# jgsimard/big-dreamer

Hardware: AMD Instinct MI355X
Metric: latent transitions/sec (RSSM + imagination) at batch=50 chunk=50 H=15 (higher is better)
Workload: dtype f32

## Files before the change

### big_dreamer_amd/csrc/wgrad.hip

```cpp
#include "bd_device.h"
#include "bd_host.h"
#include <stdint.h>
#include <stdlib.h>

namespace bd {

typedef float floatx16 __attribute__((ext_vector_type(16)));
constexpr int kWT = 64;
constexpr int kWM = 32;

__global__ __launch_bounds__(kThreads) void wgrad_kernel(const float* __restrict__ dpre, int ldp,
                                                         const float* __restrict__ act, int lda, int M, int N, int K,
                                                         int has_bias, int rows_per_split, float* __restrict__ ws) {
    __shared__ float P[kWM][kWT];
    __shared__ float A[kWM][kWT];
    const int Kext = K + has_bias;
    const int n0 = blockIdx.x * kWT, k0 = blockIdx.y * kWT;
    const int m_begin = blockIdx.z * rows_per_split;
    const int m_end = min(M, m_begin + rows_per_split);
    const int lane = threadIdx.x & 63, wave = threadIdx.x >> 6;
    const int wn = (wave >> 1) * 32, wk = (wave & 1) * 32;
    floatx16 acc;
#pragma unroll
    for (int i = 0; i < 16; ++i) acc[i] = 0.f;
    const int c = threadIdx.x & 63, r0 = threadIdx.x >> 6;
    for (int m0 = m_begin; m0 < m_end; m0 += kWM) {
        float pv[kWM / 4], av[kWM / 4];
#pragma unroll
        for (int i = 0; i < kWM / 4; ++i) {
            const int m = m0 + r0 + 4 * i;
            const bool ok = m < m_end;
            pv[i] = (ok && n0 + c < N) ? dpre[(size_t)m * ldp + n0 + c] : 0.f;
            const int k = k0 + c;
            av[i] = ok ? (k < K ? act[(size_t)m * lda + k] : (k == K && has_bias ? 1.f : 0.f)) : 0.f;
        }
        __syncthreads();
#pragma unroll
        for (int i = 0; i < kWM / 4; ++i) {
            P[r0 + 4 * i][c] = pv[i];
            A[r0 + 4 * i][c] = av[i];
        }
        __syncthreads();
#pragma unroll
        for (int s = 0; s < kWM / 2; ++s) {
            const float a = P[2 * s + (lane >> 5)][wn + (lane & 31)];
            const float b = A[2 * s + (lane >> 5)][wk + (lane & 31)];
            acc = __builtin_amdgcn_mfma_f32_32x32x2f32(a, b, acc, 0, 0, 0);
        }
    }
    float* slab = ws + (size_t)blockIdx.z * N * Kext;
    const int k = k0 + wk + (lane & 31);
#pragma unroll
    for (int reg = 0; reg < 16; ++reg) {
        const int n = n0 + wn + (reg & 3) + 8 * (reg >> 2) + 4 * (lane >> 5);
        if (n < N && k < Kext) slab[(size_t)n * Kext + k] = acc[reg];
    }
}

__global__ __launch_bounds__(256) void wgrad_reduce_kernel(const float* __restrict__ ws, int splits, int N, int K,
                                                           int has_bias, float* __restrict__ dW, int ldw,
                                                           float* __restrict__ db, int accumulate) {
    const int Kext = K + has_bias;
    const int total = N * Kext;
    for (int e = blockIdx.x * blockDim.x + threadIdx.x; e < total; e += gridDim.x * blockDim.x) {
        float s = 0.f;
        for (int z = 0; z < splits; ++z) s += ws[(size_t)z * total + e];
        const int n = e / Kext, k = e - n * Kext;
        float* dst = k < K ? dW + (size_t)n * ldw + k : db + n;
        *dst = accumulate ? *dst + s : s;
    }
}

__global__ __launch_bounds__(kThreads) void wgrad_grouped_kernel(const bd_wgrad_desc* __restrict__ descs, int n,
                                                                 float* __restrict__ ws) {
    __shared__ float P[kWM][kWT];
    __shared__ float A[kWM][kWT];
    int g = 0;
    while (g + 1 < n && (int)blockIdx.x >= descs[g + 1].block_begin) ++g;
    const bd_wgrad_desc d = descs[g];
    const int hb = d.db != nullptr;
    const int Kext = d.K + hb;
    int local = blockIdx.x - d.block_begin;
    const int z = local / (d.tiles_n * d.tiles_k);
    local -= z * d.tiles_n * d.tiles_k;
    const int n0 = (local / d.tiles_k) * kWT, k0 = (local % d.tiles_k) * kWT;
    const int m_begin = z * d.rows_per;
    const int m_end = min(d.M, m_begin + d.rows_per);
    const int lane = threadIdx.x & 63, wave = threadIdx.x >> 6;
    const int wn = (wave >> 1) * 32, wk = (wave & 1) * 32;
    floatx16 acc;
#pragma unroll
    for (int i = 0; i < 16; ++i) acc[i] = 0.f;
    const int c = threadIdx.x & 63, r0 = threadIdx.x >> 6;
    float pv[kWM / 4], av[kWM / 4];
    auto fetch = [&](int m0) {
#pragma unroll
        for (int i = 0; i < kWM / 4; ++i) {
            const int m = m0 + r0 + 4 * i;
            const bool ok = m < m_end;
            pv[i] = (ok && n0 + c < d.N) ? d.dpre[(size_t)m * d.ldp + n0 + c] : 0.f;
            const int k = k0 + c;
            float v = 0.f;
            if (ok) {
                if (k < d.K) v = m < d.M1 ? d.act1[(size_t)m * d.lda1 + k] : d.act2[(size_t)(m - d.M1) * d.lda2 + k];
                else if (k == d.K && hb) v = 1.f;
            }
            av[i] = v;
        }
    };
    fetch(m_begin);
    for (int m0 = m_begin; m0 < m_end; m0 += kWM) {
        __syncthreads();
#pragma unroll
        for (int i = 0; i < kWM / 4; ++i) {
            P[r0 + 4 * i][c] = pv[i];
            A[r0 + 4 * i][c] = av[i];
        }
        __syncthreads();
        if (m0 + kWM < m_end) fetch(m0 + kWM);
#pragma unroll
        for (int s = 0; s < kWM / 2; ++s) {
            const float a = P[2 * s + (lane >> 5)][wn + (lane & 31)];
            const float b = A[2 * s + (lane >> 5)][wk + (lane & 31)];
            acc = __builtin_amdgcn_mfma_f32_32x32x2f32(a, b, acc, 0, 0, 0);
        }
    }
    float* slab = ws + d.ws_off + (size_t)z * d.N * Kext;
    const int k = k0 + wk + (lane & 31);
#pragma unroll
    for (int reg = 0; reg < 16; ++reg) {
        const int nn = n0 + wn + (reg & 3) + 8 * (reg >> 2) + 4 * (lane >> 5);
        if (nn < d.N && k < Kext) slab[(size_t)nn * Kext + k] = acc[reg];
    }
}

constexpr int kWB = 13;
constexpr int kWBK = 12;
constexpr int kWBKDeep = 36;
__host__ __device__ __forceinline__ int wgrad_tiles_k(int NB, int KB, bool deep_ok) {
    if (KB <= kWB) return 1;
    return (NB <= 4 && deep_ok) ? cdiv(KB, kWBKDeep) : cdiv(KB, kWBK);
}
__host__ inline bool wgrad_act16(const bd_wgrad_desc& d) {
    auto al16 = [](const void* q) { return (reinterpret_cast<uintptr_t>(q) & 15) == 0; };
    if ((d.K & 3) != 0 || !al16(d.act1)) return false;
    if (d.g_nseg > 0) return (d.g_C & 3) == 0 && (d.g_seglen & 3) == 0;
    return (d.lda1 & 3) == 0 && (d.M1 == d.M || ((d.lda2 & 3) == 0 && al16(d.act2)));
}
constexpr int kWLd = 240;
constexpr int kWRows = 16;
constexpr int kWStage = 2 * kWRows * kWLd;
constexpr int kWRing = 3;
constexpr int kWRowsTall = 32;
constexpr int kWLdNarrow = 80;
constexpr int kWLdMid = 144;
constexpr int kWLdDeep = 592;
constexpr size_t kWideLdsBytes = 147456;
static_assert((size_t)kWRing * kWRows * (kWLdNarrow + kWLdDeep) * sizeof(float) <= kWideLdsBytes, "deep stage ring");
static_assert((size_t)kWRing * kWRowsTall * (kWLdMid + kWLd) * sizeof(float) <= kWideLdsBytes, "mid stage ring");
constexpr int kWThreads = 512;

template <int WN, int WK, int ROWS = kWRows, int PLD = kWLd, int ALD = kWLd>
__device__ __forceinline__ void wgrad_wide_body(const bd_wgrad_desc& d, float* __restrict__ ws, float* wlds, int hb, int Kext,
                                                int z, int n0, int k0, int nb_cnt, int kb_cnt) {
    const int m_begin = z * d.rows_per;
    const int m_end = min(d.M, m_begin + d.rows_per);
    const int lane = threadIdx.x & 63;
    const int wave = __builtin_amdgcn_readfirstlane(threadIdx.x >> 6);
    const int wr = wave & 1, wc = wave >> 1;
    const int hn = (nb_cnt + 1) >> 1;
    const int my_nb0 = wr ? hn : 0, my_nb = wr ? nb_cnt - hn : hn;
    const int kq = kb_cnt >> 2, krem = kb_cnt & 3;
    const int my_kb0 = wc * kq + min(wc, krem), my_kb = kq + (wc < krem ? 1 : 0);

    constexpr int kStage = ROWS * (PLD + ALD);
    constexpr int kRpw = ROWS / 8;
    static_assert(kWRing * kStage * sizeof(float) <= kWideLdsBytes, "stage ring exceeds the LDS request");
    floatx4 acc[WN][WK];
#pragma unroll
    for (int i = 0; i < WN; ++i)
#pragma unroll
        for (int j = 0; j < WK; ++j) acc[i][j] = floatx4{0.f, 0.f, 0.f, 0.f};

    typedef __attribute__((address_space(3))) void* lds_ptr_t;
    typedef const __attribute__((address_space(1))) void* glb_ptr_t;
    const int ncol = min(nb_cnt * 16, d.N - n0), kcol = min(kb_cnt * 16, d.K - k0);
    for (int i = threadIdx.x; i < kWRing * kStage; i += kWThreads) wlds[i] = 0.f;
    __syncthreads();
    if (hb && d.K >= k0 && d.K < k0 + kb_cnt * 16 && threadIdx.x < kWRing * ROWS)
        wlds[(threadIdx.x / ROWS) * kStage + ROWS * PLD + (threadIdx.x % ROWS) * ALD + (d.K - k0)] = 1.f;
    auto al16 = [](const void* q) { return (reinterpret_cast<uintptr_t>(q) & 15) == 0; };
    const bool p4 = (ncol & 3) == 0 && (d.ldp & 3) == 0 && al16(d.dpre + n0);
    const bool gathered = d.g_nseg > 0;
    const bool a4 = (kcol & 3) == 0 && (k0 & 3) == 0 &&
                    (gathered ? ((d.g_C & 3) == 0 && (d.g_seglen & 3) == 0 && al16(d.act1))
                              : ((d.lda1 & 3) == 0 && al16(d.act1) && (d.M1 == d.M || ((d.lda2 & 3) == 0 && al16(d.act2)))));
    constexpr int kCh4 = (ALD + 255) / 256;
    constexpr int kCh1 = (ALD + 63) / 64;
    constexpr int kGo = kCh1;
    int goff[kGo];
#pragma unroll
    for (int cc = 0; cc < kGo; ++cc) goff[cc] = 0;
    if (gathered) {
#pragma unroll
        for (int cc = 0; cc < kGo; ++cc) {
            const int k = k0 + (a4 ? 4 * lane + 256 * cc : lane + 64 * cc), sgm = k / d.g_seglen;
            goff[cc] = sgm * d.g_IW * d.g_C + (k - sgm * d.g_seglen);
        }
    }
    auto issue = [&](float* buf, int m0) {
#pragma unroll
        for (int rr = 0; rr < kRpw; ++rr) {
            const int m = m0 + wave * kRpw + rr;
            float* P = buf + (wave * kRpw + rr) * PLD;
            float* A = buf + ROWS * PLD + (wave * kRpw + rr) * ALD;
            if (m < m_end) {
                const float* prow = d.dpre + (size_t)m * d.ldp + n0;
                if (p4) {
                    if (4 * lane < ncol) __builtin_amdgcn_global_load_lds((glb_ptr_t)(prow + 4 * lane), (lds_ptr_t)P, 16, 0, 0);
                } else {
#pragma unroll
                    for (int cc = 0; cc < 4; ++cc) {
                        const int c = lane + 64 * cc;
                        if (c < ncol) __builtin_amdgcn_global_load_lds((glb_ptr_t)(prow + c), (lds_ptr_t)(P + 64 * cc), 4, 0, 0);
                    }
                }
                const float* abase;
                if (gathered) {
                    const int img = m / (d.g_gh * d.g_gw), rem = m - img * d.g_gh * d.g_gw;
                    const int y = rem / d.g_gw, x = rem - y * d.g_gw;
                    abase = d.act1 + (((size_t)img * d.g_IH + 2 * y) * d.g_IW + 2 * x) * d.g_C;
                } else {
                    abase = (m < d.M1 ? d.act1 + (size_t)m * d.lda1 : d.act2 + (size_t)(m - d.M1) * d.lda2) + k0;
                }
                if (a4) {
#pragma unroll
                    for (int cc = 0; cc < kCh4; ++cc)
                        if (4 * lane + 256 * cc < kcol)
                            __builtin_amdgcn_global_load_lds((glb_ptr_t)(abase + (gathered ? goff[cc] : 4 * lane + 256 * cc)),
                                                             (lds_ptr_t)(A + 256 * cc), 16, 0, 0);
                } else {
#pragma unroll
                    for (int cc = 0; cc < kCh1; ++cc) {
                        const int c = lane + 64 * cc;
                        if (c < kcol)
                            __builtin_amdgcn_global_load_lds((glb_ptr_t)(abase + (gathered ? goff[cc] : c)), (lds_ptr_t)(A + 64 * cc), 4,
                                                             0, 0);
                    }
                }
            } else {
#pragma unroll
                for (int cc = 0; cc < kCh1; ++cc) {
                    const int c = lane + 64 * cc;
                    if (c < PLD) P[c] = 0.f;
                    if (c < ALD) A[c] = 0.f;
                }
            }
        }
    };
    const int nst = cdiv(m_end - m_begin, ROWS);
    const int n_dma = kRpw * ((p4 ? 1 : cdiv(ncol, 64)) + (a4 ? cdiv(kcol, 256) : cdiv(kcol, 64)));
    auto wait_keep_newest = [&]() {
        switch (n_dma) {
            case 4: asm volatile("s_waitcnt vmcnt(4)" ::: "memory"); break;
            case 6: asm volatile("s_waitcnt vmcnt(6)" ::: "memory"); break;
            case 8: asm volatile("s_waitcnt vmcnt(8)" ::: "memory"); break;
            case 10: asm volatile("s_waitcnt vmcnt(10)" ::: "memory"); break;
            case 12: asm volatile("s_waitcnt vmcnt(12)" ::: "memory"); break;
            case 14: asm volatile("s_waitcnt vmcnt(14)" ::: "memory"); break;
            default: asm volatile("s_waitcnt vmcnt(16)" ::: "memory"); break;
        }
    };
    __syncthreads();
    issue(wlds, m_begin);
    if (nst > 1) issue(wlds + kStage, m_begin + ROWS);
    __builtin_amdgcn_s_waitcnt(0);
    __syncthreads();
    const int lrow = lane >> 4, lcol = lane & 15;
    for (int st = 0; st < nst; ++st) {
        const float* buf = wlds + (st % kWRing) * kStage;
        const bool more = st + 2 < nst;
        [[maybe_unused]] const int sb = (st == 10 || st == 11) ? (st - 10) * 8 : -1;
        BD_DSTAMP(sb, 0);
        if (more) issue(wlds + ((st + 2) % kWRing) * kStage, m_begin + (st + 2) * ROWS);
        BD_DSTAMP(sb, 1);
        const float* Pb = buf + lrow * PLD + my_nb0 * 16 + lcol;
        const float* Ab = buf + ROWS * PLD + lrow * ALD + my_kb0 * 16 + lcol;
#pragma unroll
        for (int sl = 0; sl < ROWS / 4; ++sl) {
            float a[WN], b[WK];
#pragma unroll
            for (int i = 0; i < WN; ++i) a[i] = Pb[sl * 4 * PLD + i * 16];
#pragma unroll
            for (int j = 0; j < WK; ++j) b[j] = Ab[sl * 4 * ALD + j * 16];
#pragma unroll
            for (int i = 0; i < WN; ++i)
#pragma unroll
                for (int j = 0; j < WK; ++j) acc[i][j] = mfma16(a[i], b[j], acc[i][j]);
        }
        BD_DSTAMP(sb, 2);
        if (more && st + 3 < nst) wait_keep_newest();
        else asm volatile("s_waitcnt vmcnt(0)" ::: "memory");
        BD_DSTAMP(sb, 3);
        lds_barrier();
        BD_DSTAMP(sb, 4);
    }
    float* slab = ws + d.ws_off + (size_t)z * d.N * Kext;
#pragma unroll
    for (int i = 0; i < WN; ++i) {
        if (i < my_nb) {
#pragma unroll
            for (int j = 0; j < WK; ++j) {
                if (j < my_kb) {
                    const int k = k0 + (my_kb0 + j) * 16 + lcol;
#pragma unroll
                    for (int r = 0; r < 4; ++r) {
                        const int nn = n0 + (my_nb0 + i) * 16 + 4 * lrow + r;
                        if (nn < d.N && k < Kext) slab[(size_t)nn * Kext + k] = acc[i][j][r];
                    }
                }
            }
        }
    }
}

template <int WN, int WK>
__device__ __forceinline__ void wgrad_dense_body(const bd_wgrad_desc& d, float* __restrict__ ws, float* wlds, int hb, int Kext,
                                                 int z, int n0, int k0, int nb_cnt, int kb_cnt, int my_nb0, int my_kb0) {
    const int m_begin = z * d.rows_per;
    const int m_end = min(d.M, m_begin + d.rows_per);
    const int lane = threadIdx.x & 63;
    const int wave = __builtin_amdgcn_readfirstlane(threadIdx.x >> 6);
    floatx4 acc[WN][WK];
#pragma unroll
    for (int i = 0; i < WN; ++i)
#pragma unroll
        for (int j = 0; j < WK; ++j) acc[i][j] = floatx4{0.f, 0.f, 0.f, 0.f};
    typedef __attribute__((address_space(3))) void* lds_ptr_t;
    typedef const __attribute__((address_space(1))) void* glb_ptr_t;
    const int ncol = min(nb_cnt * 16, d.N - n0), kcol = min(kb_cnt * 16, d.K - k0);
    for (int i = threadIdx.x; i < kWRing * kWStage; i += kWThreads) wlds[i] = 0.f;
    __syncthreads();
    if (hb && d.K >= k0 && d.K < k0 + kb_cnt * 16 && threadIdx.x < kWRing * kWRows)
        wlds[(threadIdx.x >> 4) * kWStage + kWRows * kWLd + (threadIdx.x & 15) * kWLd + (d.K - k0)] = 1.f;
    const bool lp = 4 * lane < ncol, la = 4 * lane < kcol;
    const float* __restrict__ pl = d.dpre + n0 + 4 * lane;
    const float* __restrict__ a1l = d.act1 + k0 + 4 * lane;
    const float* __restrict__ a2l = (d.M1 < d.M ? d.act2 : d.act1) + k0 + 4 * lane;
    auto issue = [&](float* buf, int m0) {
#pragma unroll
        for (int rr = 0; rr < 2; ++rr) {
            const int m = m0 + wave * 2 + rr;
            float* P = buf + (wave * 2 + rr) * kWLd;
            float* A = P + kWRows * kWLd;
            if (m < m_end) {
                if (lp) __builtin_amdgcn_global_load_lds((glb_ptr_t)(pl + (size_t)m * d.ldp), (lds_ptr_t)P, 16, 0, 0);
                const float* ar = m < d.M1 ? a1l + (size_t)m * d.lda1 : a2l + (size_t)(m - d.M1) * d.lda2;
                if (la) __builtin_amdgcn_global_load_lds((glb_ptr_t)ar, (lds_ptr_t)A, 16, 0, 0);
            } else {
#pragma unroll
                for (int cc = 0; cc < 4; ++cc) {
                    const int c = lane + 64 * cc;
                    if (c < kWLd) {
                        P[c] = 0.f;
                        A[c] = 0.f;
                    }
                }
            }
        }
    };
    const int nst = cdiv(m_end - m_begin, kWRows);
    __syncthreads();
    issue(wlds, m_begin);
    if (nst > 1) issue(wlds + kWStage, m_begin + kWRows);
    __builtin_amdgcn_s_waitcnt(0);
    __syncthreads();
    const int lrow = lane >> 4, lcol = lane & 15;
    for (int st = 0; st < nst; ++st) {
        const float* buf = wlds + (st % kWRing) * kWStage;
        const bool more = st + 2 < nst;
        [[maybe_unused]] const int sb = (st == 10 || st == 11) ? (st - 10) * 8 : -1;
        BD_DSTAMP(sb, 0);
        if (more && wave < 4) issue(wlds + ((st + 2) % kWRing) * kWStage, m_begin + (st + 2) * kWRows);
        BD_DSTAMP(sb, 1);
        const float* Pb = buf + lrow * kWLd + my_nb0 * 16 + lcol;
        const float* Ab = buf + kWRows * kWLd + lrow * kWLd + my_kb0 * 16 + lcol;
#pragma unroll
        for (int sl = 0; sl < kWRows / 4; ++sl) {
            float a[WN], b[WK];
#pragma unroll
            for (int i = 0; i < WN; ++i) a[i] = Pb[sl * 4 * kWLd + i * 16];
#pragma unroll
            for (int j = 0; j < WK; ++j) b[j] = Ab[sl * 4 * kWLd + j * 16];
#pragma unroll
            for (int i = 0; i < WN; ++i)
#pragma unroll
                for (int j = 0; j < WK; ++j) acc[i][j] = mfma16(a[i], b[j], acc[i][j]);
            if (sl == 1 && more && wave >= 4) issue(wlds + ((st + 2) % kWRing) * kWStage, m_begin + (st + 2) * kWRows);
        }
        BD_DSTAMP(sb, 2);
        if (more && st + 3 < nst) asm volatile("s_waitcnt vmcnt(4)" ::: "memory");
        else asm volatile("s_waitcnt vmcnt(0)" ::: "memory");
        BD_DSTAMP(sb, 3);
        lds_barrier();
        BD_DSTAMP(sb, 4);
    }
    float* slab = ws + d.ws_off + (size_t)z * d.N * Kext;
#pragma unroll
    for (int i = 0; i < WN; ++i) {
#pragma unroll
        for (int j = 0; j < WK; ++j) {
            const int k = k0 + (my_kb0 + j) * 16 + lcol;
#pragma unroll
            for (int r = 0; r < 4; ++r) {
                const int nn = n0 + (my_nb0 + i) * 16 + 4 * lrow + r;
                if (nn < d.N && k < Kext) slab[(size_t)nn * Kext + k] = acc[i][j][r];
            }
        }
    }
}

constexpr int kThinMaxKB = 7;
constexpr int kThinDpreFloats = 1024;
__host__ __device__ inline int thin_band_floats(int k, int roww) { return (k * roww + 64 + 255) & ~255; }
__host__ inline bool wgrad_thin_ok(const bd_wgrad_desc& d) {
    auto al16 = [](const void* q) { return (reinterpret_cast<uintptr_t>(q) & 15) == 0; };
    if (d.g_nseg <= 0 || d.g_C > 4 || d.N != 32 || d.ldp != 32 || d.g_gw > 32) return false;
    if (cdiv(d.K, 16) > kThinMaxKB || d.g_seglen != d.g_nseg * d.g_C) return false;
    const int roww = d.g_IW * d.g_C;
    if ((roww & 3) != 0 || !al16(d.act1) || !al16(d.dpre)) return false;
    const size_t per_wave = 2 * (size_t)(thin_band_floats(d.g_nseg, roww) + kThinDpreFloats) * sizeof(float);
    return 8 * per_wave <= kWideLdsBytes && (size_t)8 * 2 * kThinMaxKB * 1024 <= kWideLdsBytes;
}

#ifndef BD_WGRAD_TALL_MID
#define BD_WGRAD_TALL_MID 1
#endif
__device__ __forceinline__ bool tall_mid() { return BD_WGRAD_TALL_MID != 0; }

template <int KB>
__device__ __forceinline__ void wgrad_thin_body(const bd_wgrad_desc& d, float* __restrict__ ws, float* wlds, int z) {
    typedef __attribute__((address_space(3))) void* lds_ptr_t;
    typedef const __attribute__((address_space(1))) void* glb_ptr_t;
    const int lane = threadIdx.x & 63;
    const int wave = __builtin_amdgcn_readfirstlane(threadIdx.x >> 6);
    const int hb = d.db != nullptr;
    const int Kext = d.K + hb;
    const int gh = d.g_gh, gw = d.g_gw, C = d.g_C, kk = d.g_nseg;
    const int roww = d.g_IW * C, band = kk * roww, drow = gw * 32;
    const int band_al = thin_band_floats(kk, roww);
    const int per_buf = band_al + kThinDpreFloats;
    float* mine = wlds + (size_t)wave * 2 * per_buf;
    for (int i = lane; i < 2 * per_buf; i += 64) mine[i] = 0.f;
    asm volatile("s_waitcnt lgkmcnt(0)" ::: "memory");
    const int imgs = d.M / (gh * gw), ipw = d.rows_per / (gh * gw);
    const int img0 = z * ipw, img1 = min(imgs, img0 + ipw);
    const int items = (img1 - img0) * gh;
    const int nband = cdiv(band, 256), ndrow = cdiv(drow, 256);
    auto issue = [&](int it, float* buf) {
        const int img = img0 + it / gh, y = it - (it / gh) * gh;
        const float* sb = d.act1 + ((size_t)img * d.g_IH + 2 * y) * roww;
        const float* sd = d.dpre + ((size_t)img * gh + y) * gw * 32;
        for (int ch = 0; ch < nband; ++ch)
            if (4 * lane + 256 * ch < band)
                __builtin_amdgcn_global_load_lds((glb_ptr_t)(sb + 4 * lane + 256 * ch), (lds_ptr_t)(buf + 256 * ch), 16, 0, 0);
        for (int ch = 0; ch < ndrow; ++ch)
            if (4 * lane + 256 * ch < drow)
                __builtin_amdgcn_global_load_lds((glb_ptr_t)(sd + 4 * lane + 256 * ch), (lds_ptr_t)(buf + band_al + 256 * ch), 16, 0, 0);
    };
    const int n_dma = nband + ndrow;
    auto wait_keep_newest = [&]() {
        switch (n_dma) {
            case 5: asm volatile("s_waitcnt vmcnt(5)" ::: "memory"); break;
            case 6: asm volatile("s_waitcnt vmcnt(6)" ::: "memory"); break;
            case 7: asm volatile("s_waitcnt vmcnt(7)" ::: "memory"); break;
            case 8: asm volatile("s_waitcnt vmcnt(8)" ::: "memory"); break;
            case 9: asm volatile("s_waitcnt vmcnt(9)" ::: "memory"); break;
            case 10: asm volatile("s_waitcnt vmcnt(10)" ::: "memory"); break;
            default: asm volatile("s_waitcnt vmcnt(0)" ::: "memory"); break;
        }
    };
    int boff[KB];
    bool bok[KB];
#pragma unroll
    for (int kb = 0; kb < KB; ++kb) {
        const int kidx = kb * 16 + (lane & 15);
        bok[kb] = kidx < d.K;
        const int ky = kidx / d.g_seglen;
        boff[kb] = bok[kb] ? ky * roww + (kidx - ky * d.g_seglen) : 0;
    }
    floatx4 acc[2][KB];
#pragma unroll
    for (int i = 0; i < 2; ++i)
#pragma unroll
        for (int j = 0; j < KB; ++j) acc[i][j] = floatx4{0.f, 0.f, 0.f, 0.f};
    float bsum[2] = {0.f, 0.f};
    const int q = lane >> 4, n = lane & 15;
    const int nsl = cdiv(gw, 4);
    int it = wave, b = 0;
    if (it < items) issue(it, mine);
    for (; it < items; it += 8, b ^= 1) {
        const bool more = it + 8 < items;
        if (more) {
            issue(it + 8, mine + (b ^ 1) * per_buf);
            wait_keep_newest();
        } else {
            asm volatile("s_waitcnt vmcnt(0)" ::: "memory");
        }
        const float* Bd = mine + b * per_buf;
        const float* Dp = Bd + band_al;
        for (int sl = 0; sl < nsl; ++sl) {
            const int x = 4 * sl + q;
            const float a0 = Dp[x * 32 + n], a1 = Dp[x * 32 + 16 + n];
            float bv[KB];
#pragma unroll
            for (int kb = 0; kb < KB; ++kb) bv[kb] = bok[kb] ? Bd[boff[kb] + 2 * x * C] : 0.f;
#pragma unroll
            for (int kb = 0; kb < KB; ++kb) {
                acc[0][kb] = mfma16(a0, bv[kb], acc[0][kb]);
                acc[1][kb] = mfma16(a1, bv[kb], acc[1][kb]);
            }
            bsum[0] += a0;
            bsum[1] += a1;
        }
        asm volatile("s_waitcnt lgkmcnt(0)" ::: "memory");
    }
    __syncthreads();
    floatx4* R4 = reinterpret_cast<floatx4*>(wlds);
    float* BS = wlds + (size_t)8 * 2 * KB * 256;
#pragma unroll
    for (int i = 0; i < 2; ++i) {
#pragma unroll
        for (int j = 0; j < KB; ++j) R4[((wave * 2 + i) * KB + j) * 64 + lane] = acc[i][j];
        BS[(wave * 2 + i) * 64 + lane] = bsum[i];
    }
    __syncthreads();
    float* slab = ws + d.ws_off + (size_t)z * d.N * Kext;
    for (int e = threadIdx.x; e < 2 * KB * 64; e += blockDim.x) {
        const int blk = e >> 6, l = e & 63;
        floatx4 s4 = floatx4{0.f, 0.f, 0.f, 0.f};
        for (int w = 0; w < 8; ++w) s4 += R4[(w * 2 * KB + blk) * 64 + l];
        const int i = blk / KB, j = blk - i * KB;
        const int k = j * 16 + (l & 15);
        if (k < d.K) {
#pragma unroll
            for (int r = 0; r < 4; ++r) slab[(size_t)(i * 16 + 4 * (l >> 4) + r) * Kext + k] = s4[r];
        }
    }
    if (hb && threadIdx.x < 32) {
        const int i = threadIdx.x >> 4, nn = threadIdx.x & 15;
        float t = 0.f;
        for (int w = 0; w < 8; ++w)
            for (int qq = 0; qq < 4; ++qq) t += BS[(w * 2 + i) * 64 + qq * 16 + nn];
        slab[(size_t)(i * 16 + nn) * Kext + d.K] = t;
    }
}

__global__ __launch_bounds__(kWThreads) void wgrad_wide_kernel(const bd_wgrad_desc* __restrict__ descs, int n,
                                                         float* __restrict__ ws) {
    extern __shared__ float wlds[];
    int g = 0;
    while (g + 1 < n && (int)blockIdx.x >= descs[g + 1].block_begin) ++g;
    const bd_wgrad_desc d = descs[g];
    const int hb = d.db != nullptr;
    const int Kext = d.K + hb;
    const int NB = cdiv(d.N, 16), KB = cdiv(Kext, 16);
    const int nbw = cdiv(NB, d.tiles_n), kbw = cdiv(KB, d.tiles_k);
    int local = blockIdx.x - d.block_begin;
    const int z = local / (d.tiles_n * d.tiles_k);
    local -= z * d.tiles_n * d.tiles_k;
    const int tn = local / d.tiles_k, tk = local - tn * d.tiles_k;
    const int n0 = tn * nbw * 16, k0 = tk * kbw * 16;
    const int nb_cnt = min(nbw, NB - tn * nbw), kb_cnt = min(kbw, KB - tk * kbw);
    if (d.g_pad == 1) {
        const int kb_t = cdiv(d.K, 16);
        if (kb_t <= 3) wgrad_thin_body<3>(d, ws, wlds, z);
        else wgrad_thin_body<kThinMaxKB>(d, ws, wlds, z);
        return;
    }
    const int hn = (nb_cnt + 1) >> 1, hk = (kb_cnt + 3) >> 2;
    {
        auto al16 = [](const void* q) { return (reinterpret_cast<uintptr_t>(q) & 15) == 0; };
        const int ncol = min(nb_cnt * 16, d.N - n0), kcol = min(kb_cnt * 16, d.K - k0);
        const bool dense = nb_cnt == 13 && kb_cnt >= 4 && d.g_nseg == 0 && (ncol & 3) == 0 && (d.ldp & 3) == 0 &&
                           al16(d.dpre + n0) && (kcol & 3) == 0 && (k0 & 3) == 0 && (d.lda1 & 3) == 0 && al16(d.act1) &&
                           (d.M1 == d.M || ((d.lda2 & 3) == 0 && al16(d.act2)));
        if (dense) {
            const int wave = __builtin_amdgcn_readfirstlane(threadIdx.x >> 6);
            const int wr = (0xB2 >> wave) & 1;
            const int c = (0x13232100 >> (4 * wave)) & 3;
            const int kq = kb_cnt >> 2, krem = kb_cnt & 3;
            const int my_nb0 = wr ? 7 : 0, my_nb = wr ? 6 : 7;
            const int my_kb0 = c * kq + min(c, krem), my_kb = kq + (c < krem ? 1 : 0);
#define BD_WD(WN, WK) wgrad_dense_body<WN, WK>(d, ws, wlds, hb, Kext, z, n0, k0, nb_cnt, kb_cnt, my_nb0, my_kb0)
#define BD_WD_ROW(WN)                 \
    do {                              \
        if (my_kb == 4) BD_WD(WN, 4); \
        else if (my_kb == 3) BD_WD(WN, 3); \
        else if (my_kb == 2) BD_WD(WN, 2); \
        else BD_WD(WN, 1);            \
    } while (0)
            if (my_nb == 7) BD_WD_ROW(7);
            else BD_WD_ROW(6);
#undef BD_WD_ROW
#undef BD_WD
            return;
        }
    }
    if (nb_cnt <= 4) {
#define BD_WN_BODY(WN, WK) wgrad_wide_body<WN, WK, kWRowsTall, kWLdNarrow>(d, ws, wlds, hb, Kext, z, n0, k0, nb_cnt, kb_cnt)
#define BD_WN_ROW(WN)                      \
    do {                                   \
        if (hk <= 1) BD_WN_BODY(WN, 1);    \
        else if (hk <= 2) BD_WN_BODY(WN, 2); \
        else if (hk <= 3) BD_WN_BODY(WN, 3); \
        else BD_WN_BODY(WN, 4);            \
    } while (0)
        if (kb_cnt > 15) {
#define BD_WDEEP(WN, WK) wgrad_wide_body<WN, WK, kWRows, kWLdNarrow, kWLdDeep>(d, ws, wlds, hb, Kext, z, n0, k0, nb_cnt, kb_cnt)
            if (hn <= 1) { if (hk <= 8) BD_WDEEP(1, 8); else BD_WDEEP(1, 9); }
            else { if (hk <= 8) BD_WDEEP(2, 8); else BD_WDEEP(2, 9); }
#undef BD_WDEEP
            return;
        }
        if (hn <= 1) BD_WN_ROW(1);
        else BD_WN_ROW(2);
#undef BD_WN_ROW
#undef BD_WN_BODY
        return;
    }
    if (nb_cnt <= 8 && tall_mid()) {
#define BD_WM_BODY(WN, WK) wgrad_wide_body<WN, WK, kWRowsTall, kWLdMid>(d, ws, wlds, hb, Kext, z, n0, k0, nb_cnt, kb_cnt)
#define BD_WM_ROW(WN)                      \
    do {                                   \
        if (hk <= 1) BD_WM_BODY(WN, 1);    \
        else if (hk <= 2) BD_WM_BODY(WN, 2); \
        else if (hk <= 3) BD_WM_BODY(WN, 3); \
        else BD_WM_BODY(WN, 4);            \
    } while (0)
        if (hn <= 2) BD_WM_ROW(2);
        else BD_WM_ROW(4);
#undef BD_WM_ROW
#undef BD_WM_BODY
        return;
    }
#define BD_WG_BODY(WN, WK) wgrad_wide_body<WN, WK>(d, ws, wlds, hb, Kext, z, n0, k0, nb_cnt, kb_cnt)
#define BD_WG_ROW(WN)                      \
    do {                                   \
        if (hk <= 1) BD_WG_BODY(WN, 1);    \
        else if (hk <= 2) BD_WG_BODY(WN, 2); \
        else if (hk <= 3) BD_WG_BODY(WN, 3); \
        else BD_WG_BODY(WN, 4);            \
    } while (0)
    if (hn <= 1) BD_WG_ROW(1);
    else if (hn <= 2) BD_WG_ROW(2);
    else if (hn <= 4) BD_WG_ROW(4);
    else BD_WG_ROW(7);
#undef BD_WG_ROW
#undef BD_WG_BODY
}

__global__ __launch_bounds__(256) void wgrad_grouped_reduce_kernel(const bd_wgrad_desc* __restrict__ descs, int n,
                                                                   const float* __restrict__ ws) {
    int g = 0;
    while (g + 1 < n && (int)blockIdx.x >= descs[g + 1].red_begin) ++g;
    const bd_wgrad_desc d = descs[g];
    const int hb = d.db != nullptr;
    const int Kext = d.K + hb;
    const int total = d.N * Kext;
    const int e = (blockIdx.x - d.red_begin) * blockDim.x + threadIdx.x;
    if (e >= total) return;
    const float* p = ws + d.ws_off + e;
    float s = 0.f;
    for (int z = 0; z < d.splits; ++z) s += p[(size_t)z * total];
    const int nn = e / Kext, k = e - nn * Kext;
    if (k < d.K) d.dW[(size_t)nn * d.ldw + k] = s;
    else d.db[nn] = s;
}

#ifdef BD_STAMPS
extern "C" int bd_debug_wstamps(unsigned long long* out64) {
    return hipMemcpyFromSymbol(out64, HIP_SYMBOL(g_dstamps), sizeof(unsigned long long) * 64) == hipSuccess ? 0 : -1;
}
#endif

static bool wgrad_wide() {
    static const char* e = getenv("BD_WGRAD_WIDE");
    return !(e && e[0] == '0');
}
static bool thin_on() {
    static const char* e = getenv("BD_WGRAD_THIN");
    return !(e && e[0] == '0');
}
static int wgrad_rows() {
    static const char* e = getenv("BD_WGRAD_ROWS");
    const int r = e ? atoi(e) : 0;
    return r >= kWRows ? cdiv(r, kWRows) * kWRows : 0;
}

static void wgrad_plan(int M, int N, int K, int has_bias, int* splits, int* rows_per) {
    const int tiles = cdiv(N, kWT) * cdiv(K + has_bias, kWT);
    int s = 1024 / tiles;
    const int max_s = cdiv(M, 2 * kWM);
    if (s > max_s) s = max_s;
    if (s < 1) s = 1;
    int rp = cdiv(cdiv(M, s), kWM) * kWM;
    *rows_per = rp;
    *splits = cdiv(M, rp);
}

}

extern "C" {

int bd_wgrad_plan(bd_wgrad_desc* descs, int n, int* total_blocks, int* total_red_blocks, size_t* ws_floats) {
    using namespace bd;
    BD_REQUIRE(descs && n > 0 && total_blocks && total_red_blocks && ws_floats, "bd_wgrad_plan: bad arguments");
    int blocks = 0, red = 0;
    size_t off = 0;
    int rows_wide = wgrad_rows();
    if (wgrad_wide() && rows_wide == 0) {
        auto wgs = [&](int R) {
            long t = 0;
            for (int i = 0; i < n; ++i)
                t += (long)cdiv(cdiv(descs[i].N, 16), kWB) * wgrad_tiles_k(cdiv(descs[i].N, 16), cdiv(descs[i].K + (descs[i].db != nullptr), 16), wgrad_act16(descs[i])) *
                     cdiv(descs[i].M > 0 ? descs[i].M : 1, R);
            return t;
        };
        rows_wide = 128;
        while (wgs(rows_wide) > 256 && rows_wide < (1 << 20)) rows_wide += kWRows;
    }
    bool any_gather = false;
    for (int i = 0; i < n; ++i) any_gather = any_gather || descs[i].g_nseg > 0;
    auto tile_cost = [](int nb, int kb) {
        const int hn = (nb + 1) >> 1, kq = kb >> 2, kr = kb & 3;
        const int c = hn * ((kq + (0 < kr ? 1 : 0)) + (kq + (2 < kr ? 1 : 0)));
        return (c > 0 ? c : 1) + 12;
    };
    auto desc_geo = [&](const bd_wgrad_desc& d, int* tiles, int* cost) {
        const int NB = cdiv(d.N, 16), KB = cdiv(d.K + (d.db != nullptr), 16);
        const int tn = cdiv(NB, kWB), tk = wgrad_tiles_k(NB, KB, wgrad_act16(d));
        *tiles = tn * tk;
        *cost = tile_cost(cdiv(NB, tn), cdiv(KB, tk));
    };
    auto thin = [&](const bd_wgrad_desc& d) { return wgrad_wide() && thin_on() && wgrad_thin_ok(d); };
    auto rows_for = [&](const bd_wgrad_desc& d, double T) {
        int t, c;
        desc_geo(d, &t, &c);
        long r = (long)(T / c);
        r = (r / kWRows) * kWRows;
        return (int)(r < 4 * kWRows ? 4 * kWRows : (r > (1 << 22) ? (1 << 22) : r));
    };
    auto blocks_for = [&](double T) {
        long b = 0;
        for (int i = 0; i < n; ++i) {
            const bd_wgrad_desc& d = descs[i];
            if (thin(d)) {
                const int imgs = d.M / (d.g_gh * d.g_gw);
                b += cdiv(imgs, cdiv(imgs, 256));
                continue;
            }
            int t, c;
            desc_geo(d, &t, &c);
            b += (long)t * cdiv(d.M > 0 ? d.M : 1, rows_for(d, T));
        }
        return b;
    };
    double budget = 0.0;
    if (wgrad_wide() && any_gather) {
        double W = 0.0;
        for (int i = 0; i < n; ++i) {
            int t, c;
            desc_geo(descs[i], &t, &c);
            W += (double)t * (descs[i].M > 0 ? descs[i].M : 1) * c;
        }
        double R = W / (256.0 * 1024.0 * 61.0);
        if (R < 1.0) R = 1.0;
        if (R > 24.0) R = 24.0;
        const int rounds = (int)(R + 0.999);
        budget = W / (256.0 * (double)rounds);
        long target = 256L * rounds;
        if (blocks_for(budget * 8.0) > target) target += 256;
        for (int it = 0; it < 200 && blocks_for(budget) > target; ++it) budget *= 1.02;
    }
    for (int i = 0; i < n; ++i) {
        bd_wgrad_desc& d = descs[i];
        BD_REQUIRE(d.dpre && d.act1 && d.dW && d.M > 0 && d.N > 0 && d.K > 0 && d.M1 >= 0 && d.M1 <= d.M,
                   "bd_wgrad_plan: descriptor %d is malformed", i);
        BD_REQUIRE(d.M1 == d.M || d.act2, "bd_wgrad_plan: descriptor %d needs a second activation source", i);
        BD_REQUIRE(d.ldp >= d.N && (d.g_nseg > 0 || d.lda1 >= d.K) && d.ldw >= d.K && (d.M1 == d.M || d.lda2 >= d.K),
                   "bd_wgrad_plan: descriptor %d has a leading dimension that is too small", i);
        if (d.g_nseg > 0)
            BD_REQUIRE(wgrad_wide() && d.M1 == d.M && d.g_seglen > 0 && d.g_nseg * d.g_seglen == d.K && d.g_gh > 0 &&
                           d.g_gw > 0 && d.M % (d.g_gh * d.g_gw) == 0 && d.g_C > 0 && 2 * (d.g_gh - 1) + d.g_nseg <= d.g_IH &&
                           (2 * (d.g_gw - 1)) * d.g_C + d.g_seglen <= d.g_IW * d.g_C,
                       "bd_wgrad_plan: descriptor %d has an inconsistent gather geometry", i);
        const int hb = d.db != nullptr;
        d.g_pad = 0;
        if (wgrad_wide() && wgrad_thin_ok(d) && thin_on()) {
            const int px = d.g_gh * d.g_gw, imgs = d.M / px;
            const int ipw = cdiv(imgs, 256);
            d.g_pad = 1;
            d.tiles_n = d.tiles_k = 1;
            d.rows_per = ipw * px;
            d.splits = cdiv(imgs, ipw);
        } else if (wgrad_wide()) {
            d.tiles_n = cdiv(cdiv(d.N, 16), kWB);
            d.tiles_k = wgrad_tiles_k(cdiv(d.N, 16), cdiv(d.K + hb, 16), wgrad_act16(d));
            d.rows_per = rows_wide;
            if (budget > 0.0) d.rows_per = rows_for(d, budget);
            d.splits = cdiv(d.M, d.rows_per);
        } else {
            d.tiles_n = cdiv(d.N, kWT);
            d.tiles_k = cdiv(d.K + hb, kWT);
            int s = d.M / 512;
            if (s < 1) s = 1;
            if (s > 64) s = 64;
            d.rows_per = cdiv(cdiv(d.M, s), kWM) * kWM;
            d.splits = cdiv(d.M, d.rows_per);
        }
        d.block_begin = blocks;
        d.red_begin = red;
        d.ws_off = off;
        blocks += d.tiles_n * d.tiles_k * d.splits;
        red += cdiv(d.N * (d.K + hb), 256);
        off += (size_t)d.splits * d.N * (d.K + hb);
    }
    *total_blocks = blocks;
    *total_red_blocks = red;
    *ws_floats = off;
    return 0;
}

int bd_wgrad_grouped(const bd_wgrad_desc* descs_dev, int n, int total_blocks, int total_red_blocks, float* ws,
                     void* stream) {
    return bd_wgrad_grouped_phase(descs_dev, n, total_blocks, total_red_blocks, ws, 0, stream);
}

int bd_wgrad_grouped_phase(const bd_wgrad_desc* descs_dev, int n, int total_blocks, int total_red_blocks, float* ws,
                           int phase, void* stream) {
    using namespace bd;
    BD_REQUIRE(descs_dev && ws && n > 0 && n <= 4096 && total_blocks > 0 && total_red_blocks > 0 && phase >= 0 && phase <= 2,
               "bd_wgrad_grouped: bad arguments");
    if (phase == 2) {
    } else if (wgrad_wide()) {
        static_assert(kThreads == 256, "the 64x64-tile wgrad kernels are written for four waves");
        static bool lds_ok = false;
        if (!lds_ok) {
            if (allow_big_lds(wgrad_wide_kernel)) return -1;
            lds_ok = true;
        }
        hipLaunchKernelGGL(wgrad_wide_kernel, dim3(total_blocks), dim3(kWThreads), kWideLdsBytes, (hipStream_t)stream,
                           descs_dev, n, ws);
    } else {
        hipLaunchKernelGGL(wgrad_grouped_kernel, dim3(total_blocks), dim3(kThreads), 0, (hipStream_t)stream, descs_dev, n, ws);
    }
    BD_CHECK_LAUNCH("bd_wgrad_grouped");
    if (phase == 1) return 0;
    hipLaunchKernelGGL(wgrad_grouped_reduce_kernel, dim3(total_red_blocks), dim3(256), 0, (hipStream_t)stream, descs_dev, n,
                       ws);
    BD_CHECK_LAUNCH("bd_wgrad_grouped(reduce)");
    return 0;
}

size_t bd_wgrad_ws_floats(int M, int N, int K) {
    int s0, s1, rp;
    bd::wgrad_plan(M, N, K, 0, &s0, &rp);
    bd::wgrad_plan(M, N, K, 1, &s1, &rp);
    const size_t a = (size_t)s0 * N * K, b = (size_t)s1 * N * (K + 1);
    return a > b ? a : b;
}

int bd_wgrad(const float* dpre, int ldp, const float* act, int lda, int M, int N, int K, float* dW, int ldw,
             float* db, int accumulate, float* ws, size_t ws_floats, void* stream) {
    using namespace bd;
    BD_REQUIRE(dpre && act && dW && ws && M > 0 && N > 0 && K > 0, "bd_wgrad: bad arguments");
    BD_REQUIRE(ldp >= N && lda >= K && ldw >= K, "bd_wgrad: leading dimension too small");
    const int hb = db != nullptr;
    int splits, rows_per;
    wgrad_plan(M, N, K, hb, &splits, &rows_per);
    BD_REQUIRE((size_t)splits * N * (K + hb) <= ws_floats, "bd_wgrad: workspace too small (%zu floats, need %zu)",
               ws_floats, (size_t)splits * N * (K + hb));
    hipLaunchKernelGGL(wgrad_kernel, dim3(cdiv(N, kWT), cdiv(K + hb, kWT), splits), dim3(kThreads), 0,
                       (hipStream_t)stream, dpre, ldp, act, lda, M, N, K, hb, rows_per, ws);
    BD_CHECK_LAUNCH("bd_wgrad");
    const int total = N * (K + hb);
    hipLaunchKernelGGL(wgrad_reduce_kernel, dim3(cdiv(total, 256) < 1024 ? cdiv(total, 256) : 1024), dim3(256), 0,
                       (hipStream_t)stream, ws, splits, N, K, hb, dW, ldw, db, accumulate);
    BD_CHECK_LAUNCH("bd_wgrad(reduce)");
    return 0;
}

}
```

Before: 13.47 million.

## Pad wgrad split slabs, vectorize stores and reduce, and allow multi-round row splits

```diff
diff --git a/big_dreamer_amd/csrc/wgrad.hip b/big_dreamer_amd/csrc/wgrad.hip
--- a/big_dreamer_amd/csrc/wgrad.hip
+++ b/big_dreamer_amd/csrc/wgrad.hip
@@ -159,6 +159,9 @@
 static_assert((size_t)kWRing * kWRows * (kWLdNarrow + kWLdDeep) * sizeof(float) <= kWideLdsBytes, "deep stage ring");
 static_assert((size_t)kWRing * kWRowsTall * (kWLdMid + kWLd) * sizeof(float) <= kWideLdsBytes, "mid stage ring");
 constexpr int kWThreads = 512;
+__host__ __device__ __forceinline__ int wgrad_pitch(int Kext) { return (Kext + 3) & ~3; }
+constexpr int kWMaxRounds = 3;
+constexpr int kWUnitFloor = 256;
 
 template <int WN, int WK, int ROWS = kWRows, int PLD = kWLd, int ALD = kWLd>
 __device__ __forceinline__ void wgrad_wide_body(const bd_wgrad_desc& d, float* __restrict__ ws, float* wlds, int hb, int Kext,
@@ -305,7 +308,8 @@
         lds_barrier();
         BD_DSTAMP(sb, 4);
     }
-    float* slab = ws + d.ws_off + (size_t)z * d.N * Kext;
+    const int pitch = wgrad_pitch(Kext);
+    float* slab = ws + d.ws_off + (size_t)z * d.N * pitch;
 #pragma unroll
     for (int i = 0; i < WN; ++i) {
         if (i < my_nb) {
@@ -316,7 +320,7 @@
 #pragma unroll
                     for (int r = 0; r < 4; ++r) {
                         const int nn = n0 + (my_nb0 + i) * 16 + 4 * lrow + r;
-                        if (nn < d.N && k < Kext) slab[(size_t)nn * Kext + k] = acc[i][j][r];
+                        if (nn < d.N && k < Kext) slab[(size_t)nn * pitch + k] = acc[i][j][r];
                     }
                 }
             }
@@ -339,10 +343,6 @@
     typedef __attribute__((address_space(3))) void* lds_ptr_t;
     typedef const __attribute__((address_space(1))) void* glb_ptr_t;
     const int ncol = min(nb_cnt * 16, d.N - n0), kcol = min(kb_cnt * 16, d.K - k0);
-    for (int i = threadIdx.x; i < kWRing * kWStage; i += kWThreads) wlds[i] = 0.f;
-    __syncthreads();
-    if (hb && d.K >= k0 && d.K < k0 + kb_cnt * 16 && threadIdx.x < kWRing * kWRows)
-        wlds[(threadIdx.x >> 4) * kWStage + kWRows * kWLd + (threadIdx.x & 15) * kWLd + (d.K - k0)] = 1.f;
     const bool lp = 4 * lane < ncol, la = 4 * lane < kcol;
     const float* __restrict__ pl = d.dpre + n0 + 4 * lane;
     const float* __restrict__ a1l = d.act1 + k0 + 4 * lane;
@@ -370,9 +370,23 @@
         }
     };
     const int nst = cdiv(m_end - m_begin, kWRows);
-    __syncthreads();
     issue(wlds, m_begin);
     if (nst > 1) issue(wlds + kWStage, m_begin + kWRows);
+    {
+        const int one = (hb && d.K >= k0 && d.K < k0 + kb_cnt * 16) ? d.K - k0 : -1;
+        const int npad = nb_cnt * 16 - ncol, pad = npad + kb_cnt * 16 - kcol;
+        for (int i = threadIdx.x; i < kWRing * kWRows * pad; i += kWThreads) {
+            const int row = i / pad, c = i - row * pad;
+            float* P = wlds + (row >> 4) * kWStage + (row & 15) * kWLd;
+            if (c < npad) {
+                P[ncol + c] = 0.f;
+            } else {
+                const int kc = kcol + c - npad;
+                const bool live = row >= 2 * kWRows || m_begin + row < m_end;
+                P[kWRows * kWLd + kc] = (kc == one && live) ? 1.f : 0.f;
+            }
+        }
+    }
     __builtin_amdgcn_s_waitcnt(0);
     __syncthreads();
     const int lrow = lane >> 4, lcol = lane & 15;
@@ -405,18 +419,27 @@
         lds_barrier();
         BD_DSTAMP(sb, 4);
     }
-    float* slab = ws + d.ws_off + (size_t)z * d.N * Kext;
+    const int pitch = wgrad_pitch(Kext);
+    float* slab = ws + d.ws_off + (size_t)z * d.N * pitch;
+    constexpr int kFl = WK * 16 + 4;
+    constexpr int kQ = WK * 4;
+    float* mine = wlds + wave * (16 * (4 * 16 + 4));
+    const int kw0 = k0 + my_kb0 * 16;
 #pragma unroll
     for (int i = 0; i < WN; ++i) {
 #pragma unroll
-        for (int j = 0; j < WK; ++j) {
-            const int k = k0 + (my_kb0 + j) * 16 + lcol;
-#pragma unroll
-            for (int r = 0; r < 4; ++r) {
-                const int nn = n0 + (my_nb0 + i) * 16 + 4 * lrow + r;
-                if (nn < d.N && k < Kext) slab[(size_t)nn * Kext + k] = acc[i][j][r];
-            }
-        }
+        for (int j = 0; j < WK; ++j)
+#pragma unroll
+            for (int r = 0; r < 4; ++r) mine[(4 * lrow + r) * kFl + j * 16 + lcol] = acc[i][j][r];
+        asm volatile("s_waitcnt lgkmcnt(0)" ::: "memory");
+#pragma unroll
+        for (int t = 0; t < WK; ++t) {
+            const int idx = t * 64 + lane, row = idx / kQ, q = idx - row * kQ;
+            const floatx4 v = *reinterpret_cast<const floatx4*>(mine + row * kFl + 4 * q);
+            const int nn = n0 + (my_nb0 + i) * 16 + row, k = kw0 + 4 * q;
+            if (nn < d.N && k < pitch) *reinterpret_cast<floatx4*>(slab + (size_t)nn * pitch + k) = v;
+        }
+        asm volatile("s_waitcnt lgkmcnt(0)" ::: "memory");
     }
 }
 
@@ -535,7 +558,8 @@
         BS[(wave * 2 + i) * 64 + lane] = bsum[i];
     }
     __syncthreads();
-    float* slab = ws + d.ws_off + (size_t)z * d.N * Kext;
+    const int pitch = wgrad_pitch(Kext);
+    float* slab = ws + d.ws_off + (size_t)z * d.N * pitch;
     for (int e = threadIdx.x; e < 2 * KB * 64; e += blockDim.x) {
         const int blk = e >> 6, l = e & 63;
         floatx4 s4 = floatx4{0.f, 0.f, 0.f, 0.f};
@@ -544,7 +568,7 @@
         const int k = j * 16 + (l & 15);
         if (k < d.K) {
 #pragma unroll
-            for (int r = 0; r < 4; ++r) slab[(size_t)(i * 16 + 4 * (l >> 4) + r) * Kext + k] = s4[r];
+            for (int r = 0; r < 4; ++r) slab[(size_t)(i * 16 + 4 * (l >> 4) + r) * pitch + k] = s4[r];
         }
     }
     if (hb && threadIdx.x < 32) {
@@ -552,7 +576,7 @@
         float t = 0.f;
         for (int w = 0; w < 8; ++w)
             for (int qq = 0; qq < 4; ++qq) t += BS[(w * 2 + i) * 64 + qq * 16 + nn];
-        slab[(size_t)(i * 16 + nn) * Kext + d.K] = t;
+        slab[(size_t)(i * 16 + nn) * pitch + d.K] = t;
     }
 }
 
@@ -678,6 +702,36 @@
     else d.db[nn] = s;
 }
 
+constexpr int kRedWideThreads = 64;
+constexpr int kRedFly = 16;
+__global__ __launch_bounds__(kRedWideThreads) void wgrad_wide_reduce_kernel(const bd_wgrad_desc* __restrict__ descs, int n,
+                                                                            const float* __restrict__ ws) {
+    int g = 0;
+    while (g + 1 < n && (int)blockIdx.x >= descs[g + 1].red_begin) ++g;
+    const bd_wgrad_desc d = descs[g];
+    const int hb = d.db != nullptr;
+    const int q4 = wgrad_pitch(d.K + hb) >> 2;
+    const int total4 = d.N * q4;
+    const int e = (blockIdx.x - d.red_begin) * kRedWideThreads + threadIdx.x;
+    if (e >= total4) return;
+    const floatx4* p = reinterpret_cast<const floatx4*>(ws + d.ws_off) + e;
+    floatx4 s = floatx4{0.f, 0.f, 0.f, 0.f};
+    for (int z = 0; z < d.splits; z += kRedFly) {
+        floatx4 v[kRedFly];
+#pragma unroll
+        for (int i = 0; i < kRedFly; ++i) v[i] = p[(size_t)min(z + i, d.splits - 1) * total4];
+#pragma unroll
+        for (int i = 0; i < kRedFly; ++i)
+            if (z + i < d.splits) s += v[i];
+    }
+    const int nn = e / q4, k = (e - nn * q4) * 4;
+#pragma unroll
+    for (int r = 0; r < 4; ++r) {
+        if (k + r < d.K) d.dW[(size_t)nn * d.ldw + k + r] = s[r];
+        else if (k + r == d.K && hb) d.db[nn] = s[r];
+    }
+}
+
 #ifdef BD_STAMPS
 extern "C" int bd_debug_wstamps(unsigned long long* out64) {
     return hipMemcpyFromSymbol(out64, HIP_SYMBOL(g_dstamps), sizeof(unsigned long long) * 64) == hipSuccess ? 0 : -1;
@@ -727,8 +781,21 @@
                      cdiv(descs[i].M > 0 ? descs[i].M : 1, R);
             return t;
         };
-        rows_wide = 128;
-        while (wgs(rows_wide) > 256 && rows_wide < (1 << 20)) rows_wide += kWRows;
+        auto rows_for_rounds = [&](int k) {
+            int R = 128;
+            while (wgs(R) > 256L * k && R < (1 << 20)) R += kWRows;
+            return R;
+        };
+        rows_wide = rows_for_rounds(1);
+        bool dense = true;
+        for (int i = 0; i < n; ++i) dense = dense && descs[i].g_nseg <= 0;
+        for (int k = kWMaxRounds; dense && k > 1; --k) {
+            const int R = rows_for_rounds(k);
+            if (R >= kWUnitFloor) {
+                rows_wide = R;
+                break;
+            }
+        }
     }
     bool any_gather = false;
     for (int i = 0; i < n; ++i) any_gather = any_gather || descs[i].g_nseg > 0;
@@ -823,8 +890,14 @@
         d.red_begin = red;
         d.ws_off = off;
         blocks += d.tiles_n * d.tiles_k * d.splits;
-        red += cdiv(d.N * (d.K + hb), 256);
-        off += (size_t)d.splits * d.N * (d.K + hb);
+        if (wgrad_wide()) {
+            const int pitch = wgrad_pitch(d.K + hb);
+            red += cdiv(d.N * (pitch >> 2), kRedWideThreads);
+            off += (size_t)d.splits * d.N * pitch;
+        } else {
+            red += cdiv(d.N * (d.K + hb), 256);
+            off += (size_t)d.splits * d.N * (d.K + hb);
+        }
     }
     *total_blocks = blocks;
     *total_red_blocks = red;
@@ -842,6 +915,7 @@
     using namespace bd;
     BD_REQUIRE(descs_dev && ws && n > 0 && n <= 4096 && total_blocks > 0 && total_red_blocks > 0 && phase >= 0 && phase <= 2,
                "bd_wgrad_grouped: bad arguments");
+    BD_REQUIRE(!wgrad_wide() || (reinterpret_cast<uintptr_t>(ws) & 15) == 0, "bd_wgrad_grouped: the workspace must be 16-byte aligned");
     if (phase == 2) {
     } else if (wgrad_wide()) {
         static_assert(kThreads == 256, "the 64x64-tile wgrad kernels are written for four waves");
@@ -857,8 +931,12 @@
     }
     BD_CHECK_LAUNCH("bd_wgrad_grouped");
     if (phase == 1) return 0;
-    hipLaunchKernelGGL(wgrad_grouped_reduce_kernel, dim3(total_red_blocks), dim3(256), 0, (hipStream_t)stream, descs_dev, n,
-                       ws);
+    if (wgrad_wide())
+        hipLaunchKernelGGL(wgrad_wide_reduce_kernel, dim3(total_red_blocks), dim3(kRedWideThreads), 0, (hipStream_t)stream,
+                           descs_dev, n, ws);
+    else
+        hipLaunchKernelGGL(wgrad_grouped_reduce_kernel, dim3(total_red_blocks), dim3(256), 0, (hipStream_t)stream, descs_dev, n,
+                           ws);
     BD_CHECK_LAUNCH("bd_wgrad_grouped(reduce)");
     return 0;
 }
```

After: 13.61 million (median of 6 runs). 1.01x the previous value.
